# carlobaldassi/GaussDCA.jl

Measured on AMD Instinct MI355X. Metric: end-to-end gDCA sec + achieved Cholesky TFLOP/s, N=500 M=50k q=21, higher is better.
Workload: dtype f64

## Files before the change

### gaussdca.jl_amd/csrc/gdca_api.hip

```cpp
#include <algorithm>
#include <ctype.h>
#include <math.h>
#include <stdio.h>
#include <stdlib.h>
#include <string.h>
#include <strings.h>

#include "gdca_internal.h"
#include "gdca_launch.h"

#define MAX_EV 1024
#define N_SCRATCH 10

struct gdca_buf {
    void *p;
    size_t cap;
};

struct gdca_gate {
    hipEvent_t ev[4];
    int next, last, armed, refs;
    hipStream_t batch_stream;
};

struct score_target {
    enum { CONTACT, ENERGY, PAIR, MUTATION } kind;
    double *out;
    int score, apc;
    const int8_t *X;
    int K;
// ... 628 lines not shown
    return (x + m - 1) / m * m;
}

static gdca_status weights_stage(gdca_ctx *ctx, const int8_t *Zd, int N, int M, int q, double theta_in, int fixed_thresh,
                                 bool want_theta_only, int mark_after_theta)
{
    hipStream_t s = ctx->stream;
    gdca_dev_scalars *sc = (gdca_dev_scalars *)ctx->sc.p;
    CHK(ensure(ctx, ctx->hist, gdca_column_hist_bytes(N, M)));
    if (fixed_thresh >= 0) {
        gdca_launch_set_thresh(s, sc, fixed_thresh);
    } else {
        if (theta_in < 0.0) gdca_launch_column_hist(s, Zd, (uint32_t *)ctx->hist.p, N, M);
        gdca_launch_theta_finalize(s, (const uint32_t *)ctx->hist.p, N, M, theta_in, sc);
    }
    CHK(check_launch(ctx, "theta"));
    if (mark_after_theta >= 0) CHK(mark(ctx, mark_after_theta));
    if (want_theta_only) return GDCA_OK;

    const int Mt = (M + GDCA_HTILE - 1) / GDCA_HTILE;
    CHK(ensure(ctx, ctx->Zb, gdca_bitplane_bytes(N, M)));
    CHK(ensure(ctx, ctx->hcnt, (size_t)Mt * GDCA_HTILE * sizeof(int32_t)));
    if (!ctx->tune.force_fallback && ctx->tune.hamming_mode != 0) CHK(ensure(ctx, ctx->hcand, gdca_hamming_cand_cap(M) * 8));
    const bool fp4 = !ctx->tune.force_fallback && ctx->tune.hamming_mode == 2;
    if (fp4) CHK(ensure(ctx, ctx->himg, gdca_fp4_image_bytes(N, M)));
    CHK(ensure(ctx, ctx->nk, (size_t)M * sizeof(int32_t)));
    CHK(ensure(ctx, ctx->W, (size_t)M * sizeof(double)));
    CHK(ensure(ctx, ctx->Wfix, (size_t)M * sizeof(unsigned long long)));
    gdca_fill_async(s, ctx->hcnt.p, 0, (size_t)Mt * GDCA_HTILE * sizeof(int32_t));
    gdca_launch_bitplane_pack(s, Zd, (uint32_t *)ctx->Zb.p, N, M, q, sc);
    if (ctx->tune.force_fallback)
        gdca_launch_hamming_fallback(s, Zd, (int32_t *)ctx->hcnt.p, N, M, sc);
    else
        gdca_launch_hamming(s, (const uint32_t *)ctx->Zb.p, Zd, (int32_t *)ctx->hcnt.p, N, M, sc, ctx->tune.hamming_mode, ctx->hcand.p, fp4 ? ctx->himg.p : nullptr, ctx->tune.ham_cut);
    gdca_launch_weights(s, (const int32_t *)ctx->hcnt.p, M, gdca_fix_shift(M), (int32_t *)ctx->nk.p,
                        (double *)ctx->W.p, (unsigned long long *)ctx->Wfix.p);
    gdca_launch_meff(s, (const double *)ctx->W.p, M, sc);
    return check_launch(ctx, "weights");
}

static bool norm1_settled(const gdca_ctx *ctx, int N, int q, double pc)
{
    const double pi_cap = (1.0 - pc) + pc / (double)q;
    return pc > 0.0 && 2.0 * (double)N * pi_cap * (double)q * (double)q / pc <= ctx->tune.refine_cond && ctx->tune.refine != 1;
}

static gdca_status tally_stage(gdca_ctx *ctx, const int8_t *Zd, int N, int M, int q, const double *Meff_dev, double pc,
                               int mode, double *Pi_true_out, double *out, size_t ld, bool want_norm1 = false)
{
    hipStream_t s = ctx->stream;
    const int sdim = q - 1, n = N * sdim;
    const int shift = gdca_fix_shift(M);
    const int TJ = gdca_tally_tj(q, ctx->tune.tally_tj);
    const bool skip = gdca_tally_skip(q, TJ, ctx->tune.tally_skip, M);
    const size_t keep_list = (size_t)N * M * sizeof(uint32_t);
    if (skip) CHK(ensure(ctx, ctx->keep, keep_list + (size_t)N * sizeof(int) + N));
    CHK(ensure(ctx, ctx->Zt, (size_t)N * M + 3));
// ... 1858 lines not shown
```

### gaussdca.jl_amd/csrc/gdca_internal.h

```cpp
#pragma once

#include <hip/hip_runtime.h>
#include <stdint.h>

#include "gdca.h"

#define GDCA_TILE 128
#define GDCA_HTILE 128
#define GDCA_MAXQ 31
#define GDCA_STAMPS 20

struct gdca_dev_scalars {
    double theta;
    double Meff;
    unsigned long long pair_sum;
    int thresh;
    int info;
    int bad_symbol;
    int di_noconv;
    int ham_mode;
    int ham_cand;
    unsigned long long ham_ncand;
    unsigned long long sweep_cycles, sweep_ticks;
    double inv_norm1;
// ... 34 lines not shown
    int phased_streams;
    int refine;
    double refine_cond;
    int cholesky;
    int energy_chunk;
    int pair_chunk;
    char sweep_trace[256];
};
void gdca_tuning_from_env(gdca_tuning *t);
bool gdca_tuning_set(gdca_tuning *t, const char *key, const char *value);

void gdca_launch_relayout(hipStream_t s, const int8_t *Z, int8_t *Zt, int8_t *Zc, int N, int M, int TJ);
size_t gdca_column_hist_bytes(int N, int M);
void gdca_launch_column_hist(hipStream_t s, const int8_t *Z, uint32_t *cnt, int N, int M);
void gdca_launch_theta_finalize(hipStream_t s, const uint32_t *cnt, int N, int M, double theta_in,
                                gdca_dev_scalars *sc);
void gdca_launch_set_thresh(hipStream_t s, gdca_dev_scalars *sc, int thresh);

size_t gdca_bitplane_bytes(int N, int M);
void gdca_launch_bitplane_pack(hipStream_t s, const int8_t *Z, uint32_t *Zb, int N, int M, int q,
                               gdca_dev_scalars *sc);
size_t gdca_hamming_cand_cap(int M);
size_t gdca_fp4_image_bytes(int N, int M);
void gdca_launch_hamming_fp4_probe(hipStream_t s, const uint32_t *Zb, int N, int M, int nprobe, gdca_dev_scalars *sc);
void gdca_launch_hamming_fp4(hipStream_t s, const uint32_t *Zb, void *img, int N, int M, gdca_dev_scalars *sc, void *cand_list, unsigned cap);
void gdca_launch_hamming(hipStream_t s, const uint32_t *Zb, const int8_t *Z, int32_t *cnt, int N, int M, gdca_dev_scalars *sc, int force,
                         void *cand_list, void *fp4_img, int cut);
void gdca_launch_hamming_fallback(hipStream_t s, const int8_t *Z, int32_t *cnt, int N, int M, const gdca_dev_scalars *sc);
void gdca_launch_weights(hipStream_t s, const int32_t *cnt, int M, int fix_shift, int32_t *n_out, double *W,
                         unsigned long long *Wfix);
void gdca_launch_meff(hipStream_t s, const double *W, int M, gdca_dev_scalars *sc);
void gdca_launch_fix_weights(hipStream_t s, const double *W, int M, int fix_shift, unsigned long long *Wfix,
                             gdca_dev_scalars *sc);
int gdca_fix_shift(int M);

void gdca_launch_pi_keep(hipStream_t s, const int8_t *Zt, const unsigned long long *Wfix, unsigned long long *Pifix, uint32_t *keep,
                         int *keep_n, uint8_t *sigma, int N, int M, int q, gdca_dev_scalars *sc);
void gdca_launch_pi_finalize(hipStream_t s, const unsigned long long *Pifix, int N, int q, int fix_shift,
                             const double *Meff_dev, double pc, double *Pi_true, double *Pi_pc, double *pi_max = nullptr);
void gdca_launch_cov_norm1(hipStream_t s, const double *C, size_t ld, int N, int q, double pc, double cond_limit, gdca_dev_scalars *sc,
                           int always);
int gdca_tally_tj(int q, int tj_wanted);
bool gdca_tally_skip(int q, int TJ, int skip_wanted, int M);
void gdca_launch_pair_tally(hipStream_t s, const int8_t *Zc, const int8_t *Zt, const unsigned long long *Wfix,
                            int N, int M, int q, int fix_shift, const double *Meff_dev, double pc,
                            const double *Pi_pc, int mode, double *out, size_t ld, int TJ, const uint32_t *keep = nullptr,
                            const int *keep_n = nullptr, const uint8_t *sigma = nullptr, const unsigned long long *Pifix = nullptr);
void gdca_launch_cov_from_pij(hipStream_t s, const double *Pij, const double *Pi_pc, int N, int q, double pc, double *out, size_t ld);
// ... 81 lines not shown
```

### gaussdca.jl_amd/csrc/k_hamming.hip

```cpp
#include <algorithm>
#include <cstdlib>

#include "gdca_hamming_cut.h"
#include "gdca_internal.h"
#include "gdca_launch.h"

#define NPLANES 5
#define WCHUNK 8

size_t gdca_bitplane_bytes(int N, int M)
{
    const size_t Mt = (M + GDCA_HTILE - 1) / GDCA_HTILE, NW = (N + 31) / 32;
    return Mt * NPLANES * NW * GDCA_HTILE * sizeof(uint32_t);
}

struct k_bitplane_pack_args {
    const int8_t *Z;
    uint32_t *Zb;
    int N;
    int M;
    int NW;
    int q;
    gdca_dev_scalars *sc;
};
static inline k_bitplane_pack_args k_bitplane_pack_mk(const int8_t *Z, uint32_t *Zb, int N, int M, int NW, int q, gdca_dev_scalars *sc)
{
// ... 73 lines not shown
}

#define HAM_BOUND_PLANES 3
#define HAM_CAND_CAP 1024

__shared__ int hm_any[3];
__shared__ unsigned hm_tile_n, hm_tile_base;
__shared__ uint32_t hm_list[4][HAM_LIST_WAVE];
__shared__ int hm_wave_n[4];
__shared__ unsigned hm_alive[HAM_ALIVE_SLOTS];
#define HAM_ENT_DIST 0x3ffffu
#define HAM_NO_PAIR 0x40000000u
static_assert(sizeof(((gdca_dev_scalars *)nullptr)->ham_alive) == HAM_ALIVE_SLOTS * sizeof(unsigned), "one slot per word the probe counts");
__device__ __forceinline__ bool wg_any(bool pred, int &k)
{
    const int s = k % 3, n = (k + 1) % 3;
    ++k;
    if (threadIdx.x == 0) hm_any[n] = 0;
    if (__any(pred) && (threadIdx.x & 63) == 0) atomicOr(&hm_any[s], 1);
    __syncthreads();
    return hm_any[s] != 0;
}

#define HAM_CAND_PER_TILE 16

size_t gdca_hamming_cand_cap(int M)
{
    const long long Mt = (M + GDCA_HTILE - 1) / GDCA_HTILE;
    return (size_t)std::min<long long>(Mt * (Mt + 1) / 2 * HAM_CAND_PER_TILE + 4096, 1ll << 30);
}

struct k_hamming_refine_args {
    const int8_t *Z;
    const int2 *list;
    unsigned cap;
    int N;
    int32_t *cnt;
    const gdca_dev_scalars *sc;
};
static inline k_hamming_refine_args k_hamming_refine_mk(const int8_t *Z, const int2 *list, unsigned cap, int N, int32_t *cnt, const gdca_dev_scalars *sc)
{
    return k_hamming_refine_args{Z, list, cap, N, cnt, sc};
}
template <int CAP>
__global__ __launch_bounds__(256) void k_hamming_refine(const BatchArgs<k_hamming_refine_args, CAP> B_)
{
    GDCA_MEMBER(B_);
// ... 372 lines not shown
            if (rowc[r]) atomicAdd(&rc[ty * 8 + r], rowc[r]);
        if (!diag) {
#pragma unroll
            for (int c = 0; c < 8; ++c) {
                const int lc = (c < 4) ? (tx * 4 + c) : (64 + tx * 4 + (c - 4));
                if (colc[c]) atomicAdd(&cc[lc], colc[c]);
            }
        }
    }
    __syncthreads();
    if (tid < GDCA_HTILE) {
        const int v = rc[tid];
        if (v) atomicAdd(&cnt[I * GDCA_HTILE + tid], v);
    } else if (!diag) {
        const int v = cc[tid - GDCA_HTILE];
        if (v) atomicAdd(&cnt[J * GDCA_HTILE + tid - GDCA_HTILE], v);
    }
}

struct k_hamming_decide_args {
    gdca_dev_scalars *sc;
    long long sampled_pairs;
    int force;
    int fp4_ok;
    int NW;
    int cut;
};
static inline k_hamming_decide_args k_hamming_decide_mk(gdca_dev_scalars *sc, long long sampled_pairs, int force, int fp4_ok, int NW, int cut)
{
    return k_hamming_decide_args{sc, sampled_pairs, force, fp4_ok, NW, cut};
}
template <int CAP>
__global__ void k_hamming_decide(const BatchArgs<k_hamming_decide_args, CAP> B_)
{
    GDCA_MEMBER(B_);
    gdca_dev_scalars *sc = a_.sc;
    long long sampled_pairs = a_.sampled_pairs;
    int force = a_.force;
    if (threadIdx.x == 0 && blockIdx.x == 0) {
        const double pairs = (double)sampled_pairs;
        sc->ham_mode = force >= 0 ? force : ((a_.fp4_ok && (double)sc->ham_cand2 < 2e-3 * pairs) ? 2 : ((double)sc->ham_cand < 1e-3 * pairs ? 1 : 0));
        sc->ham_ncand = 0u;
        sc->ham_cut = a_.cut > 0 ? a_.cut : (force < 0 ? gdca_hamming_pick_cut(sc->ham_alive, pairs, a_.NW) : a_.NW);
    }
}

void gdca_launch_hamming(hipStream_t s, const uint32_t *Zb, const int8_t *Z, int32_t *cnt, int N, int M, gdca_dev_scalars *sc, int force,
                         void *cand_list, void *fp4_img, int cut)
{
    const int Mt = (M + GDCA_HTILE - 1) / GDCA_HTILE, NW = (N + 31) / 32;
    const long long ntile = (long long)Mt * (Mt + 1) / 2;
    int2 *list = (int2 *)cand_list;
    const unsigned cap = (unsigned)gdca_hamming_cand_cap(M);
    const int nprobe = (int)std::min<long long>(ntile, 192);
    if (force == 2 && !fp4_img) force = 1;
    if (force < 0 && NW <= 2) force = 0;
    if (force < 0 && ntile >= 64) {
        (gdca_launch<k_hamming_args, k_hamming<1, HAM_BOUND_PLANES, true>, k_hamming<GDCA_MAXB, HAM_BOUND_PLANES, true>>(dim3((unsigned)nprobe), dim3(256), 0, s, k_hamming_mk(Zb, cnt, NW, M, Mt, sc, list, cap)));
        if (fp4_img) gdca_launch_hamming_fp4_probe(s, Zb, N, M, nprobe, sc);
        (gdca_launch<k_hamming_decide_args, k_hamming_decide<1>, k_hamming_decide<GDCA_MAXB>>(dim3(1), dim3(1), 0, s, k_hamming_decide_mk(sc, (long long)nprobe * GDCA_HTILE * GDCA_HTILE, -1, fp4_img ? 1 : 0, NW, cut)));
    } else {
        (gdca_launch<k_hamming_decide_args, k_hamming_decide<1>, k_hamming_decide<GDCA_MAXB>>(dim3(1), dim3(1), 0, s, k_hamming_decide_mk(sc, 1ll, force < 0 ? 0 : force, 0, NW, cut)));
    }
    const bool decided = !(force < 0 && ntile >= 64);
    const int form = decided ? (force < 0 ? 0 : force) : -1;
    if (fp4_img && (form == 2 || form < 0)) gdca_launch_hamming_fp4(s, Zb, fp4_img, N, M, sc, list, cap);
    if (form == 1 || form < 0)
        (gdca_launch<k_hamming_args, k_hamming<1, HAM_BOUND_PLANES, false>, k_hamming<GDCA_MAXB, HAM_BOUND_PLANES, false>>(dim3((unsigned)ntile), dim3(256), 0, s, k_hamming_mk(Zb, cnt, NW, M, Mt, sc, list, cap)));
    if (form != 0)
        (gdca_launch<k_hamming_refine_args, k_hamming_refine<1>, k_hamming_refine<GDCA_MAXB>>(dim3(2048), dim3(256), 0, s, k_hamming_refine_mk(Z, (const int2 *)list, cap, N, cnt, (const gdca_dev_scalars *)sc)));
    (gdca_launch<k_hamming_args, k_hamming<1, NPLANES, false>, k_hamming<GDCA_MAXB, NPLANES, false>>(dim3((unsigned)ntile), dim3(256), 0, s, k_hamming_mk(Zb, cnt, NW, M, Mt, sc, list, cap)));
}

struct k_hamming_bytes_args {
    const int8_t *Z;
    int32_t *cnt;
    int N;
    int M;
    const gdca_dev_scalars *sc;
};
static inline k_hamming_bytes_args k_hamming_bytes_mk(const int8_t *Z, int32_t *cnt, int N, int M, const gdca_dev_scalars *sc)
{
    return k_hamming_bytes_args{Z, cnt, N, M, sc};
}
template <int CAP>
__global__ __launch_bounds__(256) void k_hamming_bytes(const BatchArgs<k_hamming_bytes_args, CAP> B_)
{
    GDCA_MEMBER(B_);
    const int8_t *__restrict__ Z = a_.Z;
// ... 212 lines not shown
```

### gaussdca.jl_amd/csrc/k_hamming_fp4.hip

```cpp
#include <algorithm>

#include "gdca_internal.h"
#include "gdca_launch.h"

typedef int fp4x8_t __attribute__((ext_vector_type(8)));
typedef float f32x16_t __attribute__((ext_vector_type(16)));

#define F4_TILE 256
#define F4_KC 4
#define F4_ROW (F4_KC * 32 + 16)
#define F4_OP (F4_TILE * F4_ROW)
#define F4_LDS (4 * F4_OP)

static inline int f4_entries(int NW) { return (3 * NW + 2 * F4_KC - 1) / (2 * F4_KC) * (2 * F4_KC); }
size_t gdca_fp4_image_bytes(int N, int M)
{
    const size_t NW = (size_t)(N + 31) / 32, rows = ((size_t)M + F4_TILE - 1) / F4_TILE * F4_TILE;
    return rows * (size_t)f4_entries((int)NW) * 16;
}

__device__ __forceinline__ uint32_t f4_spread8(uint32_t b)
{
    uint32_t x = b & 0xffu;
    x = (x | (x << 12)) & 0x000f000fu;
    x = (x | (x << 6)) & 0x03030303u;
    x = (x | (x << 3)) & 0x11111111u;
    return (x << 3) | 0x22222222u;
}

struct k_fp4_image_args {
    const uint32_t *Zb;
    uint4 *img;
    int NW, M, E;
    const gdca_dev_scalars *sc;
};
template <int CAP>
__global__ __launch_bounds__(256) void k_fp4_image(const BatchArgs<k_fp4_image_args, CAP> B_)
{
    GDCA_MEMBER(B_);
    if (a_.sc->ham_mode != 2) return;
    const uint32_t *__restrict__ Zb = a_.Zb;
    uint4 *__restrict__ img = a_.img;
    const int NW = a_.NW, M = a_.M, E = a_.E;
    const int k = blockIdx.x * 256 + threadIdx.x, e = blockIdx.y;
    const int w = e / 3, p = e - 3 * w;
    uint4 v = make_uint4(0u, 0u, 0u, 0u);
    if (k < M && e < 3 * NW) {
        const uint32_t word = Zb[(((size_t)(k >> 7) * 5 + p) * NW + w) * 128 + (k & 127)];
        v = make_uint4(f4_spread8(word), f4_spread8(word >> 8), f4_spread8(word >> 16), f4_spread8(word >> 24));
    }
    img[(size_t)k * E + e] = v;
}

__device__ __forceinline__ void f4_tri_decode(int t, int Mt, int &I, int &J)
{
    const double b = 2.0 * Mt + 1.0;
    int i = (int)((b - sqrt(b * b - 8.0 * (double)t)) * 0.5);
    i = max(0, min(i, Mt - 1));
    auto start = [Mt](int r) { return (long long)r * Mt - (long long)r * (r - 1) / 2; };
    while (i > 0 && start(i) > t) --i;
    while (i < Mt - 1 && start(i + 1) <= t) ++i;
    I = i;
    J = i + (int)(t - start(i));
}

struct k_hamming_fp4_args {
    const unsigned char *img;
    int E, M, Mt, NW;
    gdca_dev_scalars *sc;
    int2 *cand_list;
    unsigned cand_cap;
};
__shared__ unsigned f4_tile_n, f4_tile_base;
template <int CAP>
__global__ __launch_bounds__(1024) void k_hamming_fp4(const BatchArgs<k_hamming_fp4_args, CAP> B_)
{
    GDCA_MEMBER(B_);
    gdca_dev_scalars *__restrict__ sc = a_.sc;
    if (sc->ham_mode != 2) return;
    const int thresh = sc->thresh;
    if (thresh <= 0) return;
    const unsigned char *__restrict__ img = a_.img;
    const int E = a_.E, M = a_.M, Mt = a_.Mt, NW = a_.NW;
    int2 *__restrict__ cand_list = a_.cand_list;
    const unsigned cand_cap = a_.cand_cap;
    extern __shared__ __attribute__((aligned(16))) unsigned char f4_lds[];

    int I, J;
    f4_tri_decode((int)blockIdx.x, Mt, I, J);
    const int tid = threadIdx.x, lane = tid & 63, wv = tid >> 6, wr = wv & 3, wc = wv >> 2;
    const int l32 = lane & 31, lh = lane >> 5;
    if (tid == 0) f4_tile_n = 0u;
    const size_t rowbytes = (size_t)E * 16;
    const int nchunk = E / (2 * F4_KC);

    const int srow = tid >> 3, spc = tid & 7;
    const unsigned char *ga = img + ((size_t)I * F4_TILE + srow) * rowbytes + spc * 16, *gb = img + ((size_t)J * F4_TILE + srow) * rowbytes + spc * 16;
    const size_t half = (size_t)128 * rowbytes;
    unsigned char *la = f4_lds + srow * F4_ROW + spc * 16;
    uint4 s0, s1, s2, s3;
#define F4_LOAD(ch)                                                                       \
    do {                                                                                  \
        s0 = *reinterpret_cast<const uint4 *>(ga + (size_t)(ch) * (32 * F4_KC));          \
        s1 = *reinterpret_cast<const uint4 *>(ga + half + (size_t)(ch) * (32 * F4_KC));   \
        s2 = *reinterpret_cast<const uint4 *>(gb + (size_t)(ch) * (32 * F4_KC));          \
        s3 = *reinterpret_cast<const uint4 *>(gb + half + (size_t)(ch) * (32 * F4_KC));   \
    } while (0)
#define F4_STORE(buf)                                                                     \
    do {                                                                                  \
        unsigned char *d_ = la + (size_t)(2 * (buf)) * F4_OP;                             \
        *reinterpret_cast<uint4 *>(d_) = s0;                                              \
        *reinterpret_cast<uint4 *>(d_ + 128 * F4_ROW) = s1;                               \
        *reinterpret_cast<uint4 *>(d_ + F4_OP) = s2;                                      \
        *reinterpret_cast<uint4 *>(d_ + F4_OP + 128 * F4_ROW) = s3;                       \
    } while (0)

    f32x16_t acc[2][2];
#pragma unroll
    for (int i = 0; i < 2; ++i)
#pragma unroll
        for (int j = 0; j < 2; ++j)
#pragma unroll
            for (int e = 0; e < 16; ++e) acc[i][j][e] = 0.f;
    const int one = 0x7f7f7f7f;

    const unsigned char *abase = f4_lds + (wr * 64 + l32) * F4_ROW + lh * 16, *bbase = f4_lds + F4_OP + (wc * 64 + l32) * F4_ROW + lh * 16;
    F4_LOAD(0);
    F4_STORE(0);
    __syncthreads();
    for (int ch = 0; ch < nchunk; ++ch) {
        const int buf = ch & 1;
        if (ch + 1 < nchunk) F4_LOAD(ch + 1);
        const unsigned char *As = abase + (size_t)(2 * buf) * F4_OP, *Bs = bbase + (size_t)(2 * buf) * F4_OP;
#pragma unroll 1
        for (int ks = 0; ks < F4_KC; ++ks) {
            fp4x8_t a[2], b[2];
#pragma unroll
            for (int i = 0; i < 2; ++i) {
                const uint4 x = *reinterpret_cast<const uint4 *>(As + i * 32 * F4_ROW + ks * 32);
                a[i] = (fp4x8_t){(int)x.x, (int)x.y, (int)x.z, (int)x.w, 0, 0, 0, 0};
            }
#pragma unroll
            for (int j = 0; j < 2; ++j) {
                const uint4 x = *reinterpret_cast<const uint4 *>(Bs + j * 32 * F4_ROW + ks * 32);
                b[j] = (fp4x8_t){(int)x.x, (int)x.y, (int)x.z, (int)x.w, 0, 0, 0, 0};
            }
#pragma unroll
            for (int i = 0; i < 2; ++i)
#pragma unroll
                for (int j = 0; j < 2; ++j)
                    acc[i][j] = __builtin_amdgcn_mfma_scale_f32_32x32x64_f8f6f4(a[i], b[j], acc[i][j], 4, 4, 0, one, 0, one);
        }
        if (ch + 1 < nchunk) F4_STORE(buf ^ 1);
        __syncthreads();
    }

    const float limit = (float)(96 * NW - 6 * thresh);
    const bool diag = I == J;
    unsigned mine = 0;
    unsigned long long cand[2] = {0ull, 0ull};
    float mx = acc[0][0][0];
#pragma unroll
    for (int i = 0; i < 2; ++i)
#pragma unroll
        for (int j = 0; j < 2; ++j)
#pragma unroll
            for (int e = 0; e < 16; ++e) mx = fmaxf(mx, acc[i][j][e]);
    if (mx > limit) {
#pragma unroll
        for (int i = 0; i < 2; ++i)
#pragma unroll
            for (int j = 0; j < 2; ++j) {
                const int gc = J * F4_TILE + wc * 64 + j * 32 + l32;
#pragma unroll
                for (int e = 0; e < 16; ++e) {
                    const int gr = I * F4_TILE + wr * 64 + i * 32 + 8 * (e >> 2) + 4 * lh + (e & 3);
                    if (acc[i][j][e] > limit && gr < M && gc < M && (diag ? gr < gc : true)) {
                        cand[i] |= 1ull << (16 * j + e);
                        ++mine;
                    }
                }
            }
    }
    const unsigned off = mine ? atomicAdd(&f4_tile_n, mine) : 0u;
    __syncthreads();
    if (f4_tile_n == 0u) return;
    if (tid == 0) {
        const unsigned long long base = atomicAdd(&sc->ham_ncand, (unsigned long long)f4_tile_n);
        f4_tile_base = base > (unsigned long long)cand_cap ? cand_cap : (unsigned)base;
    }
    __syncthreads();
    unsigned slot = f4_tile_base + off;
#pragma unroll
    for (int i = 0; i < 2; ++i) {
        unsigned long long c = cand[i];
        while (c) {
            const int bit = __builtin_ctzll(c), j = bit >> 4, e = bit & 15;
            const int gr = I * F4_TILE + wr * 64 + i * 32 + 8 * (e >> 2) + 4 * lh + (e & 3);
            const int gc = J * F4_TILE + wc * 64 + j * 32 + l32;
            if (slot < cand_cap) cand_list[slot] = make_int2(gr, gc);
            ++slot;
            c &= c - 1;
        }
    }
}

struct k_fp4_probe_args {
    const uint32_t *Zb;
    int NW, M, Mt;
    gdca_dev_scalars *sc;
};
template <int CAP>
__global__ __launch_bounds__(256) void k_fp4_probe(const BatchArgs<k_fp4_probe_args, CAP> B_)
{
    GDCA_MEMBER(B_);
    const uint32_t *__restrict__ Zb = a_.Zb;
    const int NW = a_.NW, M = a_.M, Mt = a_.Mt;
    gdca_dev_scalars *sc = a_.sc;
    const int thresh = sc->thresh;
    if (thresh <= 0) return;
    __shared__ int total;
    int I, J;
    f4_tri_decode((int)(((long long)blockIdx.x * ((long long)Mt * (Mt + 1) / 2)) / gridDim.x), Mt, I, J);
    const int tid = threadIdx.x, tx = tid & 15, ty = tid >> 4;
    if (tid == 0) total = 0;
    __syncthreads();
    int D[8][8];
#pragma unroll
    for (int r = 0; r < 8; ++r)
#pragma unroll
        for (int c = 0; c < 8; ++c) D[r][c] = 0;
    const uint32_t *Ag = Zb + (size_t)I * 5 * NW * 128, *Bg = Zb + (size_t)J * 5 * NW * 128;
    for (int w = 0; w < NW; ++w)
#pragma unroll
        for (int p = 0; p < 3; ++p) {
            uint32_t a[8], b[8];
#pragma unroll
            for (int r = 0; r < 8; ++r) a[r] = Ag[((size_t)p * NW + w) * 128 + ty * 8 + r];
#pragma unroll
            for (int c = 0; c < 8; ++c) b[c] = Bg[((size_t)p * NW + w) * 128 + tx * 8 + c];
#pragma unroll
            for (int r = 0; r < 8; ++r)
#pragma unroll
                for (int c = 0; c < 8; ++c) D[r][c] += __builtin_popcount(a[r] ^ b[c]);
        }
    int cand = 0;
#pragma unroll
    for (int r = 0; r < 8; ++r)
#pragma unroll
        for (int c = 0; c < 8; ++c) {
            const int gr = I * 128 + ty * 8 + r, gc = J * 128 + tx * 8 + c;
            cand += (gr < M) && (gc < M) && (gr != gc) && (D[r][c] < 3 * thresh);
        }
    if (cand) atomicAdd(&total, cand);
    __syncthreads();
    if (tid == 0 && total) atomicAdd(&sc->ham_cand2, total);
}

void gdca_launch_hamming_fp4_probe(hipStream_t s, const uint32_t *Zb, int N, int M, int nprobe, gdca_dev_scalars *sc)
{
    const int NW = (N + 31) / 32, Mt = (M + 127) / 128;
    gdca_launch<k_fp4_probe_args, k_fp4_probe<1>, k_fp4_probe<GDCA_MAXB>>(dim3((unsigned)nprobe), dim3(256), 0, s, k_fp4_probe_args{Zb, NW, M, Mt, sc});
}

void gdca_launch_hamming_fp4(hipStream_t s, const uint32_t *Zb, void *img, int N, int M, gdca_dev_scalars *sc, void *cand_list, unsigned cap)
{
    const int NW = (N + 31) / 32, E = f4_entries(NW), Mt = (M + F4_TILE - 1) / F4_TILE;
    const long long ntile = (long long)Mt * (Mt + 1) / 2;
    gdca_launch<k_fp4_image_args, k_fp4_image<1>, k_fp4_image<GDCA_MAXB>>(dim3((unsigned)Mt, (unsigned)E), dim3(256), 0, s,
                                                                           k_fp4_image_args{Zb, (uint4 *)img, NW, M, E, sc});
    gdca_launch<k_hamming_fp4_args, k_hamming_fp4<1>, k_hamming_fp4<GDCA_MAXB>>(dim3((unsigned)ntile), dim3(1024), F4_LDS, s,
                                                                                 k_hamming_fp4_args{(const unsigned char *)img, E, M, Mt, NW, sc, (int2 *)cand_list, cap});
}
```

Measured before the change: 49.25.

## Add consensus-based fp4 Hamming form with cost-model selection and segmented tiles

Replaces the three-bitplane fp4 image with a one-bit-per-site image that encodes whether each residue differs from the column consensus. The consensus is taken from the column histogram. The matmul-style candidate filter therefore runs on a third of the entries. The fp4 kernel now walks a segment of column tiles per block, so each row tile is staged once, and the fp4 path is enabled by default for large problems. A cost model picks between the dense, bound and consensus forms from probe counts. The risks are a looser consensus bound producing more candidates to refine, and the extra launches for the histogram and image.

Result: faster. 51.98, median of 6 (+5.6%).

```diff
diff --git a/gaussdca.jl_amd/csrc/gdca_api.hip b/gaussdca.jl_amd/csrc/gdca_api.hip
--- a/gaussdca.jl_amd/csrc/gdca_api.hip
+++ b/gaussdca.jl_amd/csrc/gdca_api.hip
@@ -6,6 +6,7 @@
 #include <string.h>
 #include <strings.h>
 
+#include "gdca_hamming_form.h"
 #include "gdca_internal.h"
 #include "gdca_launch.h"
 
@@ -680,17 +681,22 @@
     CHK(ensure(ctx, ctx->Zb, gdca_bitplane_bytes(N, M)));
     CHK(ensure(ctx, ctx->hcnt, (size_t)Mt * GDCA_HTILE * sizeof(int32_t)));
     if (!ctx->tune.force_fallback && ctx->tune.hamming_mode != 0) CHK(ensure(ctx, ctx->hcand, gdca_hamming_cand_cap(M) * 8));
-    const bool fp4 = !ctx->tune.force_fallback && ctx->tune.hamming_mode == 2;
+    const bool fp4 = !ctx->tune.force_fallback && (ctx->tune.hamming_mode == 2 || (ctx->tune.hamming_mode < 0 && gdca_hamming_consensus_gate(N, M)));
     if (fp4) CHK(ensure(ctx, ctx->himg, gdca_fp4_image_bytes(N, M)));
     CHK(ensure(ctx, ctx->nk, (size_t)M * sizeof(int32_t)));
     CHK(ensure(ctx, ctx->W, (size_t)M * sizeof(double)));
     CHK(ensure(ctx, ctx->Wfix, (size_t)M * sizeof(unsigned long long)));
     gdca_fill_async(s, ctx->hcnt.p, 0, (size_t)Mt * GDCA_HTILE * sizeof(int32_t));
     gdca_launch_bitplane_pack(s, Zd, (uint32_t *)ctx->Zb.p, N, M, q, sc);
-    if (ctx->tune.force_fallback)
+    if (ctx->tune.force_fallback) {
         gdca_launch_hamming_fallback(s, Zd, (int32_t *)ctx->hcnt.p, N, M, sc);
-    else
+    } else {
+        if (fp4) {
+            if (!(fixed_thresh < 0 && theta_in < 0.0)) gdca_launch_column_hist(s, Zd, (uint32_t *)ctx->hist.p, N, M);
+            gdca_launch_hamming_fp4_image(s, Zd, (const uint32_t *)ctx->hist.p, ctx->himg.p, N, M);
+        }
         gdca_launch_hamming(s, (const uint32_t *)ctx->Zb.p, Zd, (int32_t *)ctx->hcnt.p, N, M, sc, ctx->tune.hamming_mode, ctx->hcand.p, fp4 ? ctx->himg.p : nullptr, ctx->tune.ham_cut);
+    }
     gdca_launch_weights(s, (const int32_t *)ctx->hcnt.p, M, gdca_fix_shift(M), (int32_t *)ctx->nk.p,
                         (double *)ctx->W.p, (unsigned long long *)ctx->Wfix.p);
     gdca_launch_meff(s, (const double *)ctx->W.p, M, sc);
diff --git a/gaussdca.jl_amd/csrc/gdca_hamming_form.h b/gaussdca.jl_amd/csrc/gdca_hamming_form.h
--- /dev/null
+++ b/gaussdca.jl_amd/csrc/gdca_hamming_form.h
@@ -0,0 +1,50 @@
+#pragma once
+
+#if defined(__HIPCC__)
+#define GDCA_FORM_HD __host__ __device__
+#else
+#define GDCA_FORM_HD
+#endif
+
+#define HAM_CAND_PER_TILE 64
+#define HAM_FORM_MAX_DENSITY (0.5 * HAM_CAND_PER_TILE / 16384.0)
+
+#define HAM_FORM_BOUND3_DENSITY 1e-3
+
+#define HAM_T_DENSE 1.9e-3
+#define HAM_CUT_TAIL 0.35
+#define HAM_T_PAIR 0.7e-4
+#define HAM_T_REFINE 1.3e-7
+#define HAM_T_TILE 6.5e-3
+#define HAM_T_ENTRY 1.6e-4
+#define HAM_T_IMAGE 4.0e-5
+#define HAM_T_FIXED 25.0
+
+#define HAM_FORM_MIN_WORK 65536.0
+
+static inline GDCA_FORM_HD double gdca_hamming_tiles(int M)
+{
+    const double Mt = (double)((M + 127) / 128);
+    return 0.5 * Mt * (Mt + 1.0);
+}
+
+static inline GDCA_FORM_HD int gdca_hamming_consensus_gate(int N, int M)
+{
+    const int NW = (N + 31) / 32;
+    return NW > 2 && gdca_hamming_tiles(M) * (double)NW >= HAM_FORM_MIN_WORK;
+}
+
+static inline GDCA_FORM_HD int gdca_hamming_pick_form(double cand3, double cand1, double pairs, int N, int M, int cut)
+{
+    if (!(pairs > 0.0)) return 0;
+    const int NW = (N + 31) / 32;
+    const double tiles = gdca_hamming_tiles(M), all = 0.5 * (double)M * (double)M;
+    const double f3 = cand3 / pairs, f1 = cand1 / pairs;
+    const int other = f3 < HAM_FORM_BOUND3_DENSITY ? 1 : 0;
+    if (cand1 < 0.0 || f1 > HAM_FORM_MAX_DENSITY) return other;
+    const double weff = (cut > 0 && cut < NW) ? (double)cut + HAM_CUT_TAIL * (double)(NW - cut) : (double)NW;
+    const double E = (double)((NW + 7) / 8 * 8), pair = HAM_T_PAIR + (double)N * HAM_T_REFINE;
+    const double cost_other = other ? tiles * weff * HAM_T_DENSE + f3 * all * pair : tiles * (double)NW * 1.5 * HAM_T_DENSE;
+    const double cost_cons = tiles * (HAM_T_TILE + E * HAM_T_ENTRY) + f1 * all * pair + (double)M * E * HAM_T_IMAGE + HAM_T_FIXED;
+    return cost_cons < cost_other ? 2 : other;
+}
diff --git a/gaussdca.jl_amd/csrc/gdca_internal.h b/gaussdca.jl_amd/csrc/gdca_internal.h
--- a/gaussdca.jl_amd/csrc/gdca_internal.h
+++ b/gaussdca.jl_amd/csrc/gdca_internal.h
@@ -80,8 +80,9 @@
                                gdca_dev_scalars *sc);
 size_t gdca_hamming_cand_cap(int M);
 size_t gdca_fp4_image_bytes(int N, int M);
-void gdca_launch_hamming_fp4_probe(hipStream_t s, const uint32_t *Zb, int N, int M, int nprobe, gdca_dev_scalars *sc);
-void gdca_launch_hamming_fp4(hipStream_t s, const uint32_t *Zb, void *img, int N, int M, gdca_dev_scalars *sc, void *cand_list, unsigned cap);
+void gdca_launch_hamming_fp4_image(hipStream_t s, const int8_t *Z, const uint32_t *hist, void *img, int N, int M);
+void gdca_launch_hamming_fp4_probe(hipStream_t s, const void *img, int N, int M, int nprobe, gdca_dev_scalars *sc);
+void gdca_launch_hamming_fp4(hipStream_t s, const void *img, int N, int M, gdca_dev_scalars *sc, void *cand_list, unsigned cap);
 void gdca_launch_hamming(hipStream_t s, const uint32_t *Zb, const int8_t *Z, int32_t *cnt, int N, int M, gdca_dev_scalars *sc, int force,
                          void *cand_list, void *fp4_img, int cut);
 void gdca_launch_hamming_fallback(hipStream_t s, const int8_t *Z, int32_t *cnt, int N, int M, const gdca_dev_scalars *sc);
diff --git a/gaussdca.jl_amd/csrc/k_hamming.hip b/gaussdca.jl_amd/csrc/k_hamming.hip
--- a/gaussdca.jl_amd/csrc/k_hamming.hip
+++ b/gaussdca.jl_amd/csrc/k_hamming.hip
@@ -2,6 +2,7 @@
 #include <cstdlib>
 
 #include "gdca_hamming_cut.h"
+#include "gdca_hamming_form.h"
 #include "gdca_internal.h"
 #include "gdca_launch.h"
 
@@ -121,7 +122,6 @@
     return hm_any[s] != 0;
 }
 
-#define HAM_CAND_PER_TILE 16
 
 size_t gdca_hamming_cand_cap(int M)
 {
@@ -540,13 +540,13 @@
     gdca_dev_scalars *sc;
     long long sampled_pairs;
     int force;
-    int fp4_ok;
-    int NW;
+    int consensus;
+    int N, M;
     int cut;
 };
-static inline k_hamming_decide_args k_hamming_decide_mk(gdca_dev_scalars *sc, long long sampled_pairs, int force, int fp4_ok, int NW, int cut)
-{
-    return k_hamming_decide_args{sc, sampled_pairs, force, fp4_ok, NW, cut};
+static inline k_hamming_decide_args k_hamming_decide_mk(gdca_dev_scalars *sc, long long sampled_pairs, int force, int consensus, int N, int M, int cut)
+{
+    return k_hamming_decide_args{sc, sampled_pairs, force, consensus, N, M, cut};
 }
 template <int CAP>
 __global__ void k_hamming_decide(const BatchArgs<k_hamming_decide_args, CAP> B_)
@@ -557,9 +557,11 @@
     int force = a_.force;
     if (threadIdx.x == 0 && blockIdx.x == 0) {
         const double pairs = (double)sampled_pairs;
-        sc->ham_mode = force >= 0 ? force : ((a_.fp4_ok && (double)sc->ham_cand2 < 2e-3 * pairs) ? 2 : ((double)sc->ham_cand < 1e-3 * pairs ? 1 : 0));
+        const int NW = (a_.N + 31) / 32;
+        const int cut = a_.cut > 0 ? a_.cut : (force < 0 ? gdca_hamming_pick_cut(sc->ham_alive, pairs, NW) : NW);
+        sc->ham_cut = cut;
+        sc->ham_mode = force >= 0 ? force : gdca_hamming_pick_form((double)sc->ham_cand, a_.consensus ? (double)sc->ham_cand2 : -1.0, pairs, a_.N, a_.M, cut);
         sc->ham_ncand = 0u;
-        sc->ham_cut = a_.cut > 0 ? a_.cut : (force < 0 ? gdca_hamming_pick_cut(sc->ham_alive, pairs, a_.NW) : a_.NW);
     }
 }
 
@@ -575,14 +577,14 @@
     if (force < 0 && NW <= 2) force = 0;
     if (force < 0 && ntile >= 64) {
         (gdca_launch<k_hamming_args, k_hamming<1, HAM_BOUND_PLANES, true>, k_hamming<GDCA_MAXB, HAM_BOUND_PLANES, true>>(dim3((unsigned)nprobe), dim3(256), 0, s, k_hamming_mk(Zb, cnt, NW, M, Mt, sc, list, cap)));
-        if (fp4_img) gdca_launch_hamming_fp4_probe(s, Zb, N, M, nprobe, sc);
-        (gdca_launch<k_hamming_decide_args, k_hamming_decide<1>, k_hamming_decide<GDCA_MAXB>>(dim3(1), dim3(1), 0, s, k_hamming_decide_mk(sc, (long long)nprobe * GDCA_HTILE * GDCA_HTILE, -1, fp4_img ? 1 : 0, NW, cut)));
+        if (fp4_img) gdca_launch_hamming_fp4_probe(s, fp4_img, N, M, nprobe, sc);
+        (gdca_launch<k_hamming_decide_args, k_hamming_decide<1>, k_hamming_decide<GDCA_MAXB>>(dim3(1), dim3(1), 0, s, k_hamming_decide_mk(sc, (long long)nprobe * GDCA_HTILE * GDCA_HTILE, -1, fp4_img ? 1 : 0, N, M, cut)));
     } else {
-        (gdca_launch<k_hamming_decide_args, k_hamming_decide<1>, k_hamming_decide<GDCA_MAXB>>(dim3(1), dim3(1), 0, s, k_hamming_decide_mk(sc, 1ll, force < 0 ? 0 : force, 0, NW, cut)));
+        (gdca_launch<k_hamming_decide_args, k_hamming_decide<1>, k_hamming_decide<GDCA_MAXB>>(dim3(1), dim3(1), 0, s, k_hamming_decide_mk(sc, 1ll, force < 0 ? 0 : force, 0, N, M, cut)));
     }
     const bool decided = !(force < 0 && ntile >= 64);
     const int form = decided ? (force < 0 ? 0 : force) : -1;
-    if (fp4_img && (form == 2 || form < 0)) gdca_launch_hamming_fp4(s, Zb, fp4_img, N, M, sc, list, cap);
+    if (fp4_img && (form == 2 || form < 0)) gdca_launch_hamming_fp4(s, fp4_img, N, M, sc, list, cap);
     if (form == 1 || form < 0)
         (gdca_launch<k_hamming_args, k_hamming<1, HAM_BOUND_PLANES, false>, k_hamming<GDCA_MAXB, HAM_BOUND_PLANES, false>>(dim3((unsigned)ntile), dim3(256), 0, s, k_hamming_mk(Zb, cnt, NW, M, Mt, sc, list, cap)));
     if (form != 0)
diff --git a/gaussdca.jl_amd/csrc/k_hamming_fp4.hip b/gaussdca.jl_amd/csrc/k_hamming_fp4.hip
--- a/gaussdca.jl_amd/csrc/k_hamming_fp4.hip
+++ b/gaussdca.jl_amd/csrc/k_hamming_fp4.hip
@@ -11,12 +11,17 @@
 #define F4_ROW (F4_KC * 32 + 16)
 #define F4_OP (F4_TILE * F4_ROW)
 #define F4_LDS (4 * F4_OP)
-
-static inline int f4_entries(int NW) { return (3 * NW + 2 * F4_KC - 1) / (2 * F4_KC) * (2 * F4_KC); }
-size_t gdca_fp4_image_bytes(int N, int M)
+#define F4_SEG 8
+
+static inline int f4_entries(int NW) { return (NW + 2 * F4_KC - 1) / (2 * F4_KC) * (2 * F4_KC); }
+static inline size_t f4_image_only_bytes(int N, int M)
 {
     const size_t NW = (size_t)(N + 31) / 32, rows = ((size_t)M + F4_TILE - 1) / F4_TILE * F4_TILE;
     return rows * (size_t)f4_entries((int)NW) * 16;
+}
+size_t gdca_fp4_image_bytes(int N, int M)
+{
+    return f4_image_only_bytes(N, M) + (size_t)f4_entries((N + 31) / 32) * 32;
 }
 
 __device__ __forceinline__ uint32_t f4_spread8(uint32_t b)
@@ -25,31 +30,89 @@
     x = (x | (x << 12)) & 0x000f000fu;
     x = (x | (x << 6)) & 0x03030303u;
     x = (x | (x << 3)) & 0x11111111u;
-    return (x << 3) | 0x22222222u;
+    return x;
+}
+__device__ __forceinline__ uint32_t f4_nibbles8(uint32_t differs, uint32_t valid)
+{
+    return ((f4_spread8(differs) << 3) | 0x22222222u) & (f4_spread8(valid) * 0xfu);
+}
+__device__ __forceinline__ uint32_t f4_signs8(uint32_t v)
+{
+    uint32_t x = (v >> 3) & 0x11111111u;
+    x = (x | (x >> 3)) & 0x03030303u;
+    x = (x | (x >> 6)) & 0x000f000fu;
+    x = (x | (x >> 12)) & 0xffu;
+    return x;
+}
+
+struct k_fp4_sigma_args {
+    const uint32_t *hist;
+    uint8_t *sigma;
+    int N, NP;
+};
+template <int CAP>
+__global__ __launch_bounds__(256) void k_fp4_sigma(const BatchArgs<k_fp4_sigma_args, CAP> B_)
+{
+    GDCA_MEMBER(B_);
+    const uint32_t *__restrict__ hist = a_.hist;
+    const int i = blockIdx.x * 256 + threadIdx.x;
+    if (i >= a_.NP) return;
+    uint32_t best = 0u, bz = 0u;
+    if (i < a_.N) {
+        const uint4 *h = reinterpret_cast<const uint4 *>(hist + (size_t)i * 32);
+#pragma unroll
+        for (int g = 0; g < 8; ++g) {
+            const uint4 v = h[g];
+            const uint32_t c[4] = {v.x, v.y, v.z, v.w};
+#pragma unroll
+            for (int j = 0; j < 4; ++j)
+                if (c[j] > best) {
+                    best = c[j];
+                    bz = (uint32_t)(4 * g + j);
+                }
+        }
+    }
+    a_.sigma[i] = (uint8_t)bz;
 }
 
 struct k_fp4_image_args {
-    const uint32_t *Zb;
+    const int8_t *Z;
+    const uint8_t *sigma;
     uint4 *img;
-    int NW, M, E;
-    const gdca_dev_scalars *sc;
+    int N, M, E, rows;
 };
 template <int CAP>
 __global__ __launch_bounds__(256) void k_fp4_image(const BatchArgs<k_fp4_image_args, CAP> B_)
 {
     GDCA_MEMBER(B_);
-    if (a_.sc->ham_mode != 2) return;
-    const uint32_t *__restrict__ Zb = a_.Zb;
+    const int8_t *__restrict__ Z = a_.Z;
+    const uint8_t *__restrict__ sigma = a_.sigma;
     uint4 *__restrict__ img = a_.img;
-    const int NW = a_.NW, M = a_.M, E = a_.E;
-    const int k = blockIdx.x * 256 + threadIdx.x, e = blockIdx.y;
-    const int w = e / 3, p = e - 3 * w;
-    uint4 v = make_uint4(0u, 0u, 0u, 0u);
-    if (k < M && e < 3 * NW) {
-        const uint32_t word = Zb[(((size_t)(k >> 7) * 5 + p) * NW + w) * 128 + (k & 127)];
-        v = make_uint4(f4_spread8(word), f4_spread8(word >> 8), f4_spread8(word >> 16), f4_spread8(word >> 24));
-    }
-    img[(size_t)k * E + e] = v;
+    const int N = a_.N, M = a_.M, E = a_.E;
+    const long long g = (long long)blockIdx.x * 256 + threadIdx.x;
+    if (g >= (long long)a_.rows * E) return;
+    const int k = (int)(g / E), w = (int)(g - (long long)k * E);
+    uint32_t diff = 0u, valid = 0u;
+    const int nb = min(32, N - w * 32);
+    if (k < M && nb > 0) {
+        const int8_t *src = Z + (size_t)k * N + (size_t)w * 32;
+        valid = nb == 32 ? 0xffffffffu : ((1u << nb) - 1u);
+        if (nb == 32 && (N & 3) == 0 && (reinterpret_cast<uintptr_t>(Z) & 3) == 0) {
+            const uint32_t *s4 = reinterpret_cast<const uint32_t *>(src), *g4 = reinterpret_cast<const uint32_t *>(sigma + w * 32);
+#pragma unroll
+            for (int j = 0; j < 8; ++j) {
+                uint32_t x = (s4[j] & 0x1f1f1f1fu) ^ g4[j];
+                x |= x >> 4;
+                x |= x >> 2;
+                x |= x >> 1;
+                x &= 0x01010101u;
+                diff |= (((x * 0x01020408u) >> 24) & 0xfu) << (4 * j);
+            }
+        } else {
+            for (int b = 0; b < nb; ++b) diff |= (uint32_t)(((uint32_t)(uint8_t)src[b] & 31u) != (uint32_t)sigma[w * 32 + b]) << b;
+        }
+    }
+    img[g] = make_uint4(f4_nibbles8(diff, valid), f4_nibbles8(diff >> 8, valid >> 8), f4_nibbles8(diff >> 16, valid >> 16), f4_nibbles8(diff >> 24, valid >> 24));
 }
 
 __device__ __forceinline__ void f4_tri_decode(int t, int Mt, int &I, int &J)
@@ -66,13 +129,13 @@
 
 struct k_hamming_fp4_args {
     const unsigned char *img;
-    int E, M, Mt, NW;
+    int E, M, Mt, N;
     gdca_dev_scalars *sc;
     int2 *cand_list;
     unsigned cand_cap;
 };
-__shared__ unsigned f4_tile_n, f4_tile_base;
-template <int CAP>
+__shared__ unsigned f4_tile_n[2], f4_tile_base;
+template <int CAP, bool ARES>
 __global__ __launch_bounds__(1024) void k_hamming_fp4(const BatchArgs<k_hamming_fp4_args, CAP> B_)
 {
     GDCA_MEMBER(B_);
@@ -81,38 +144,53 @@
     const int thresh = sc->thresh;
     if (thresh <= 0) return;
     const unsigned char *__restrict__ img = a_.img;
-    const int E = a_.E, M = a_.M, Mt = a_.Mt, NW = a_.NW;
+    const int E = a_.E, M = a_.M, Mt = a_.Mt;
     int2 *__restrict__ cand_list = a_.cand_list;
     const unsigned cand_cap = a_.cand_cap;
     extern __shared__ __attribute__((aligned(16))) unsigned char f4_lds[];
 
-    int I, J;
-    f4_tri_decode((int)blockIdx.x, Mt, I, J);
+    const int I = (int)blockIdx.y, J0 = I + (int)blockIdx.x * F4_SEG;
+    if (J0 >= Mt) return;
+    const int J1 = min(Mt, J0 + F4_SEG);
     const int tid = threadIdx.x, lane = tid & 63, wv = tid >> 6, wr = wv & 3, wc = wv >> 2;
     const int l32 = lane & 31, lh = lane >> 5;
-    if (tid == 0) f4_tile_n = 0u;
+    if (tid == 0) {
+        f4_tile_n[0] = 0u;
+        f4_tile_n[1] = 0u;
+    }
     const size_t rowbytes = (size_t)E * 16;
     const int nchunk = E / (2 * F4_KC);
+    const int total = (J1 - J0) * nchunk;
 
     const int srow = tid >> 3, spc = tid & 7;
-    const unsigned char *ga = img + ((size_t)I * F4_TILE + srow) * rowbytes + spc * 16, *gb = img + ((size_t)J * F4_TILE + srow) * rowbytes + spc * 16;
-    const size_t half = (size_t)128 * rowbytes;
+    const unsigned char *ga = img + ((size_t)I * F4_TILE + srow) * rowbytes + spc * 16;
+    const unsigned char *gb0 = img + (size_t)srow * rowbytes + spc * 16;
+    const size_t half = (size_t)128 * rowbytes, tilebytes = (size_t)F4_TILE * rowbytes;
     unsigned char *la = f4_lds + srow * F4_ROW + spc * 16;
     uint4 s0, s1, s2, s3;
-#define F4_LOAD(ch)                                                                       \
+    s0 = s1 = make_uint4(0u, 0u, 0u, 0u);
+#define F4_LOAD_A(ch)                                                                     \
     do {                                                                                  \
         s0 = *reinterpret_cast<const uint4 *>(ga + (size_t)(ch) * (32 * F4_KC));          \
         s1 = *reinterpret_cast<const uint4 *>(ga + half + (size_t)(ch) * (32 * F4_KC));   \
-        s2 = *reinterpret_cast<const uint4 *>(gb + (size_t)(ch) * (32 * F4_KC));          \
-        s3 = *reinterpret_cast<const uint4 *>(gb + half + (size_t)(ch) * (32 * F4_KC));   \
     } while (0)
-#define F4_STORE(buf)                                                                     \
+#define F4_LOAD_B(J, ch)                                                                                      \
+    do {                                                                                                      \
+        const unsigned char *g_ = gb0 + (size_t)(J) * tilebytes + (size_t)(ch) * (32 * F4_KC);                \
+        s2 = *reinterpret_cast<const uint4 *>(g_);                                                            \
+        s3 = *reinterpret_cast<const uint4 *>(g_ + half);                                                     \
+    } while (0)
+#define F4_STORE_A(region)                                                                \
     do {                                                                                  \
-        unsigned char *d_ = la + (size_t)(2 * (buf)) * F4_OP;                             \
+        unsigned char *d_ = la + (size_t)(region) * F4_OP;                                \
         *reinterpret_cast<uint4 *>(d_) = s0;                                              \
         *reinterpret_cast<uint4 *>(d_ + 128 * F4_ROW) = s1;                               \
-        *reinterpret_cast<uint4 *>(d_ + F4_OP) = s2;                                      \
-        *reinterpret_cast<uint4 *>(d_ + F4_OP + 128 * F4_ROW) = s3;                       \
+    } while (0)
+#define F4_STORE_B(buf)                                                                   \
+    do {                                                                                  \
+        unsigned char *d_ = la + (size_t)(2 + (buf)) * F4_OP;                             \
+        *reinterpret_cast<uint4 *>(d_) = s2;                                              \
+        *reinterpret_cast<uint4 *>(d_ + 128 * F4_ROW) = s3;                               \
     } while (0)
 
     f32x16_t acc[2][2];
@@ -124,14 +202,34 @@
             for (int e = 0; e < 16; ++e) acc[i][j][e] = 0.f;
     const int one = 0x7f7f7f7f;
 
-    const unsigned char *abase = f4_lds + (wr * 64 + l32) * F4_ROW + lh * 16, *bbase = f4_lds + F4_OP + (wc * 64 + l32) * F4_ROW + lh * 16;
-    F4_LOAD(0);
-    F4_STORE(0);
+    const unsigned char *abase = f4_lds + (wr * 64 + l32) * F4_ROW + lh * 16, *bbase = f4_lds + 2 * F4_OP + (wc * 64 + l32) * F4_ROW + lh * 16;
+    const float limit = (float)(a_.N - 2 * thresh);
+
+    if constexpr (ARES) {
+        F4_LOAD_A(0);
+        F4_STORE_A(0);
+        if (nchunk > 1) {
+            F4_LOAD_A(1);
+            F4_STORE_A(1);
+        }
+    } else {
+        F4_LOAD_A(0);
+        F4_STORE_A(0);
+    }
+    F4_LOAD_B(J0, 0);
+    F4_STORE_B(0);
     __syncthreads();
-    for (int ch = 0; ch < nchunk; ++ch) {
-        const int buf = ch & 1;
-        if (ch + 1 < nchunk) F4_LOAD(ch + 1);
-        const unsigned char *As = abase + (size_t)(2 * buf) * F4_OP, *Bs = bbase + (size_t)(2 * buf) * F4_OP;
+    int J = J0, ch = 0;
+    for (int it = 0; it < total; ++it) {
+        const int buf = it & 1;
+        const bool more = it + 1 < total;
+        const bool last = ch + 1 == nchunk;
+        const int Jn = last ? J + 1 : J, chn = last ? 0 : ch + 1;
+        if (more) {
+            if constexpr (!ARES) F4_LOAD_A(chn);
+            F4_LOAD_B(Jn, chn);
+        }
+        const unsigned char *As = abase + (size_t)(ARES ? ch : buf) * F4_OP, *Bs = bbase + (size_t)buf * F4_OP;
 #pragma unroll 1
         for (int ks = 0; ks < F4_KC; ++ks) {
             fp4x8_t a[2], b[2];
@@ -151,124 +249,164 @@
                 for (int j = 0; j < 2; ++j)
                     acc[i][j] = __builtin_amdgcn_mfma_scale_f32_32x32x64_f8f6f4(a[i], b[j], acc[i][j], 4, 4, 0, one, 0, one);
         }
-        if (ch + 1 < nchunk) F4_STORE(buf ^ 1);
-        __syncthreads();
-    }
-
-    const float limit = (float)(96 * NW - 6 * thresh);
-    const bool diag = I == J;
-    unsigned mine = 0;
-    unsigned long long cand[2] = {0ull, 0ull};
-    float mx = acc[0][0][0];
-#pragma unroll
-    for (int i = 0; i < 2; ++i)
-#pragma unroll
-        for (int j = 0; j < 2; ++j)
-#pragma unroll
-            for (int e = 0; e < 16; ++e) mx = fmaxf(mx, acc[i][j][e]);
-    if (mx > limit) {
-#pragma unroll
-        for (int i = 0; i < 2; ++i)
-#pragma unroll
-            for (int j = 0; j < 2; ++j) {
-                const int gc = J * F4_TILE + wc * 64 + j * 32 + l32;
-#pragma unroll
-                for (int e = 0; e < 16; ++e) {
-                    const int gr = I * F4_TILE + wr * 64 + i * 32 + 8 * (e >> 2) + 4 * lh + (e & 3);
-                    if (acc[i][j][e] > limit && gr < M && gc < M && (diag ? gr < gc : true)) {
-                        cand[i] |= 1ull << (16 * j + e);
-                        ++mine;
+        if (more) {
+            if constexpr (!ARES) F4_STORE_A(buf ^ 1);
+            F4_STORE_B(buf ^ 1);
+        }
+        if (last) {
+            const int slot_n = (J - J0) & 1;
+            const bool diag = I == J;
+            unsigned mine = 0;
+            unsigned long long cand[2] = {0ull, 0ull};
+            float mx = acc[0][0][0];
+#pragma unroll
+            for (int i = 0; i < 2; ++i)
+#pragma unroll
+                for (int j = 0; j < 2; ++j)
+#pragma unroll
+                    for (int e = 0; e < 16; ++e) mx = fmaxf(mx, acc[i][j][e]);
+            if (mx > limit) {
+#pragma unroll
+                for (int i = 0; i < 2; ++i)
+#pragma unroll
+                    for (int j = 0; j < 2; ++j) {
+                        const int gc = J * F4_TILE + wc * 64 + j * 32 + l32;
+#pragma unroll
+                        for (int e = 0; e < 16; ++e) {
+                            const int gr = I * F4_TILE + wr * 64 + i * 32 + 8 * (e >> 2) + 4 * lh + (e & 3);
+                            if (acc[i][j][e] > limit && gr < M && gc < M && (diag ? gr < gc : true)) {
+                                cand[i] |= 1ull << (16 * j + e);
+                                ++mine;
+                            }
+                        }
+                    }
+            }
+#pragma unroll
+            for (int i = 0; i < 2; ++i)
+#pragma unroll
+                for (int j = 0; j < 2; ++j)
+#pragma unroll
+                    for (int e = 0; e < 16; ++e) acc[i][j][e] = 0.f;
+            const unsigned off = mine ? atomicAdd(&f4_tile_n[slot_n], mine) : 0u;
+            __syncthreads();
+            const unsigned ntile = f4_tile_n[slot_n];
+            if (tid == 0) f4_tile_n[slot_n ^ 1] = 0u;
+            if (ntile != 0u) {
+                if (tid == 0) {
+                    const unsigned long long base = atomicAdd(&sc->ham_ncand, (unsigned long long)ntile);
+                    f4_tile_base = base > (unsigned long long)cand_cap ? cand_cap : (unsigned)base;
+                }
+                __syncthreads();
+                unsigned slot = f4_tile_base + off;
+#pragma unroll
+                for (int i = 0; i < 2; ++i) {
+                    unsigned long long c = cand[i];
+                    while (c) {
+                        const int bit = __builtin_ctzll(c), j = bit >> 4, e = bit & 15;
+                        const int gr = I * F4_TILE + wr * 64 + i * 32 + 8 * (e >> 2) + 4 * lh + (e & 3);
+                        const int gc = J * F4_TILE + wc * 64 + j * 32 + l32;
+                        if (slot < cand_cap) cand_list[slot] = make_int2(gr, gc);
+                        ++slot;
+                        c &= c - 1;
                     }
                 }
             }
-    }
-    const unsigned off = mine ? atomicAdd(&f4_tile_n, mine) : 0u;
-    __syncthreads();
-    if (f4_tile_n == 0u) return;
-    if (tid == 0) {
-        const unsigned long long base = atomicAdd(&sc->ham_ncand, (unsigned long long)f4_tile_n);
-        f4_tile_base = base > (unsigned long long)cand_cap ? cand_cap : (unsigned)base;
-    }
-    __syncthreads();
-    unsigned slot = f4_tile_base + off;
-#pragma unroll
-    for (int i = 0; i < 2; ++i) {
-        unsigned long long c = cand[i];
-        while (c) {
-            const int bit = __builtin_ctzll(c), j = bit >> 4, e = bit & 15;
-            const int gr = I * F4_TILE + wr * 64 + i * 32 + 8 * (e >> 2) + 4 * lh + (e & 3);
-            const int gc = J * F4_TILE + wc * 64 + j * 32 + l32;
-            if (slot < cand_cap) cand_list[slot] = make_int2(gr, gc);
-            ++slot;
-            c &= c - 1;
-        }
-    }
-}
-
+        }
+        J = Jn;
+        ch = chn;
+        __syncthreads();
+    }
+}
+
+#define F4_PW 8
 struct k_fp4_probe_args {
-    const uint32_t *Zb;
-    int NW, M, Mt;
+    const uint4 *img;
+    int E, NW, M, Mt;
     gdca_dev_scalars *sc;
 };
 template <int CAP>
 __global__ __launch_bounds__(256) void k_fp4_probe(const BatchArgs<k_fp4_probe_args, CAP> B_)
 {
     GDCA_MEMBER(B_);
-    const uint32_t *__restrict__ Zb = a_.Zb;
-    const int NW = a_.NW, M = a_.M, Mt = a_.Mt;
+    const uint4 *__restrict__ img = a_.img;
+    const int E = a_.E, NW = a_.NW, M = a_.M, Mt = a_.Mt;
     gdca_dev_scalars *sc = a_.sc;
     const int thresh = sc->thresh;
     if (thresh <= 0) return;
     __shared__ int total;
+    __shared__ uint32_t bits[2][F4_PW][128];
     int I, J;
     f4_tri_decode((int)(((long long)blockIdx.x * ((long long)Mt * (Mt + 1) / 2)) / gridDim.x), Mt, I, J);
     const int tid = threadIdx.x, tx = tid & 15, ty = tid >> 4;
     if (tid == 0) total = 0;
-    __syncthreads();
     int D[8][8];
 #pragma unroll
     for (int r = 0; r < 8; ++r)
 #pragma unroll
         for (int c = 0; c < 8; ++c) D[r][c] = 0;
-    const uint32_t *Ag = Zb + (size_t)I * 5 * NW * 128, *Bg = Zb + (size_t)J * 5 * NW * 128;
-    for (int w = 0; w < NW; ++w)
-#pragma unroll
-        for (int p = 0; p < 3; ++p) {
+    const uint4 *mine = img + (size_t)((tid < 128 ? I : J) * 128 + (tid & 127)) * E;
+    for (int w0 = 0; w0 < NW; w0 += F4_PW) {
+        __syncthreads();
+#pragma unroll
+        for (int u = 0; u < F4_PW; ++u) {
+            uint32_t b = 0u;
+            if (w0 + u < NW) {
+                const uint4 v = mine[w0 + u];
+                b = f4_signs8(v.x) | (f4_signs8(v.y) << 8) | (f4_signs8(v.z) << 16) | (f4_signs8(v.w) << 24);
+            }
+            bits[tid >> 7][u][tid & 127] = b;
+        }
+        __syncthreads();
+        const int wn = min(F4_PW, NW - w0);
+        for (int u = 0; u < wn; ++u) {
             uint32_t a[8], b[8];
 #pragma unroll
-            for (int r = 0; r < 8; ++r) a[r] = Ag[((size_t)p * NW + w) * 128 + ty * 8 + r];
-#pragma unroll
-            for (int c = 0; c < 8; ++c) b[c] = Bg[((size_t)p * NW + w) * 128 + tx * 8 + c];
+            for (int r = 0; r < 8; ++r) a[r] = bits[0][u][ty * 8 + r];
+#pragma unroll
+            for (int c = 0; c < 8; ++c) b[c] = bits[1][u][tx * 8 + c];
 #pragma unroll
             for (int r = 0; r < 8; ++r)
 #pragma unroll
                 for (int c = 0; c < 8; ++c) D[r][c] += __builtin_popcount(a[r] ^ b[c]);
         }
+    }
     int cand = 0;
 #pragma unroll
     for (int r = 0; r < 8; ++r)
 #pragma unroll
         for (int c = 0; c < 8; ++c) {
             const int gr = I * 128 + ty * 8 + r, gc = J * 128 + tx * 8 + c;
-            cand += (gr < M) && (gc < M) && (gr != gc) && (D[r][c] < 3 * thresh);
+            cand += (gr < M) && (gc < M) && (gr != gc) && (D[r][c] < thresh);
         }
     if (cand) atomicAdd(&total, cand);
     __syncthreads();
     if (tid == 0 && total) atomicAdd(&sc->ham_cand2, total);
 }
 
-void gdca_launch_hamming_fp4_probe(hipStream_t s, const uint32_t *Zb, int N, int M, int nprobe, gdca_dev_scalars *sc)
+void gdca_launch_hamming_fp4_image(hipStream_t s, const int8_t *Z, const uint32_t *hist, void *img, int N, int M)
+{
+    const int NW = (N + 31) / 32, E = f4_entries(NW), rows = (M + F4_TILE - 1) / F4_TILE * F4_TILE;
+    uint8_t *sigma = (uint8_t *)img + f4_image_only_bytes(N, M);
+    gdca_launch<k_fp4_sigma_args, k_fp4_sigma<1>, k_fp4_sigma<GDCA_MAXB>>(dim3((unsigned)((32 * E + 255) / 256)), dim3(256), 0, s, k_fp4_sigma_args{hist, sigma, N, 32 * E});
+    const long long items = (long long)rows * E;
+    gdca_launch<k_fp4_image_args, k_fp4_image<1>, k_fp4_image<GDCA_MAXB>>(dim3((unsigned)((items + 255) / 256)), dim3(256), 0, s,
+                                                                           k_fp4_image_args{Z, sigma, (uint4 *)img, N, M, E, rows});
+}
+
+void gdca_launch_hamming_fp4_probe(hipStream_t s, const void *img, int N, int M, int nprobe, gdca_dev_scalars *sc)
 {
     const int NW = (N + 31) / 32, Mt = (M + 127) / 128;
-    gdca_launch<k_fp4_probe_args, k_fp4_probe<1>, k_fp4_probe<GDCA_MAXB>>(dim3((unsigned)nprobe), dim3(256), 0, s, k_fp4_probe_args{Zb, NW, M, Mt, sc});
-}
-
-void gdca_launch_hamming_fp4(hipStream_t s, const uint32_t *Zb, void *img, int N, int M, gdca_dev_scalars *sc, void *cand_list, unsigned cap)
+    gdca_launch<k_fp4_probe_args, k_fp4_probe<1>, k_fp4_probe<GDCA_MAXB>>(dim3((unsigned)nprobe), dim3(256), 0, s,
+                                                                           k_fp4_probe_args{(const uint4 *)img, f4_entries(NW), NW, M, Mt, sc});
+}
+
+void gdca_launch_hamming_fp4(hipStream_t s, const void *img, int N, int M, gdca_dev_scalars *sc, void *cand_list, unsigned cap)
 {
     const int NW = (N + 31) / 32, E = f4_entries(NW), Mt = (M + F4_TILE - 1) / F4_TILE;
-    const long long ntile = (long long)Mt * (Mt + 1) / 2;
-    gdca_launch<k_fp4_image_args, k_fp4_image<1>, k_fp4_image<GDCA_MAXB>>(dim3((unsigned)Mt, (unsigned)E), dim3(256), 0, s,
-                                                                           k_fp4_image_args{Zb, (uint4 *)img, NW, M, E, sc});
-    gdca_launch<k_hamming_fp4_args, k_hamming_fp4<1>, k_hamming_fp4<GDCA_MAXB>>(dim3((unsigned)ntile), dim3(1024), F4_LDS, s,
-                                                                                 k_hamming_fp4_args{(const unsigned char *)img, E, M, Mt, NW, sc, (int2 *)cand_list, cap});
-}
+    const dim3 grid((unsigned)((Mt + F4_SEG - 1) / F4_SEG), (unsigned)Mt);
+    const k_hamming_fp4_args a{(const unsigned char *)img, E, M, Mt, N, sc, (int2 *)cand_list, cap};
+    if (E <= 4 * F4_KC)
+        gdca_launch<k_hamming_fp4_args, k_hamming_fp4<1, true>, k_hamming_fp4<GDCA_MAXB, true>>(grid, dim3(1024), F4_LDS, s, a);
+    else
+        gdca_launch<k_hamming_fp4_args, k_hamming_fp4<1, false>, k_hamming_fp4<GDCA_MAXB, false>>(grid, dim3(1024), F4_LDS, s, a);
+}
```
